# eliotwang/SageAttention

Hardware: AMD Instinct MI355X
Metric: attention fwd TFLOPS at head_dim=128 seqlen=8192 (INT8 QK^T + FP16 PV, quantizers included) (higher is better)
Workload: dtype int8+fp16; 1 GPU; c3: qk_int8_pv_fp16 (B,H,N,D)=(4,32,8192,128) causal=False qk_quant_gran=per_thread; global_batch=4, seq_len=8192, head_dim=128, heads=32, parallelism=single

## Files before the change

### sageattention_amd/csrc/sage_entry.h

```cpp
#pragma once
#include "sage_attn_common.h"

namespace sage {

struct QuantParams {
  const uint16_t* x;
  int64_t xsb, xsh, xsn;
  const uint16_t* mean;
  int8_t* out;
  int64_t osb, osh, osn;
  float* scale;
  const uint16_t* dot_vec;
  float* dot_out;
  int dot_group;
  int N, G;
  int gran, is_key;
  int warp;
  int warp_shift;
  float mult;
  int rounding;
  const int* cu;
  int64_t o_blk, ss_b, ss_h, ss_blk;
  const float* mean_part;
  int S;
  uint16_t* km_out;
};

struct VPrepParams {
  const uint16_t* v;
  int64_t sb, sh, sn;
  uint8_t* out;
  int64_t ob, oh, od, o_tile;
  float* v_scale;
  const float* part;
  float scale_max;
};

struct QuantOptions {
  const int* cu = nullptr;
  int64_t out_blk_stride = 0;
  const int64_t* scale_strides = nullptr;
  const float* mean_part = nullptr;
  int S = 0;
  void* km_out = nullptr;
};

struct QuantCall {
  QuantParams p;
  int B, H, D, blk;
  bool bf16;
};
int quant_check(QuantCall& c, const sage_tensor* x, int dtype, int B, int H, int N, int D, const void* mean,
                const sage_tensor* out, float* scale, int gran, int is_key, int blk, int warp, float mult, int rounding,
                const void* lse_dot_vec, int dot_group, float* lse_dot, const QuantOptions& opt = QuantOptions());
int quant_launch(const QuantCall& c, hipStream_t st);

struct KSmoothCall {
  QuantCall q;
  sage_tensor k;
  float* part;
  int per_wg;
  const int32_t* kv_lens = nullptr;
};
int k_smooth_quant_check(KSmoothCall& c, const sage_tensor* k, int dtype, int B, int H, int N, int D, const sage_tensor* out,
                         float* scale, void* km, int gran, int rounding, void* workspace, const int32_t* kv_lens = nullptr);
int k_smooth_quant_launch(const KSmoothCall& c, hipStream_t st);

struct KVPrepCall {
  QuantCall k;
  VPrepParams v;
  float* kpart;
  float* vpart;
  int nblk_k, nunit_v;
  int per_k, per_v;
  bool streaming;
  const int32_t* kv_lens = nullptr;
};
int kv_prepare_check(KVPrepCall& c, const sage_tensor* k, const sage_tensor* v, int dtype, int B, int H, int N, int D,
                     const sage_tensor* k_int8, float* k_scale, void* km, int gran, int rounding, const sage_tensor* v_fp8,
                     float* v_scale, float scale_max, void* workspace,
                     const int32_t* kv_lens = nullptr);
int kv_prepare_launch(const KVPrepCall& c, hipStream_t st);

struct AttnArgs {
  const sage_tensor *q = nullptr, *k8 = nullptr, *v = nullptr, *o = nullptr;
  bool pv_fp8 = false;
  int v_dtype = SAGE_F16, o_dtype = SAGE_F16;
  const float *q_scale = nullptr, *k_scale = nullptr, *v_scale = nullptr, *v_mean = nullptr;
  float* lse = nullptr;
  int B = 0, Hq = 0, Hk = 0, M = 0, N = 0, D = 0;
  int is_causal = 0, qk_gran = 0, blkq = 0, warpq = 0;
  float sm_scale = 0.f;
  int logit_mult_is_one = 0;
  const int *cu_q = nullptr, *cu_k = nullptr;
  int q_dtype = -1;
  const void* km = nullptr;
  const void* mask = nullptr;
  int mask_kind = 0;
  const int64_t* mask_strides = nullptr;
  const sage_kv_layout* kvl = nullptr;
  int nwaves = 0;
  bool block_sparse = false;
  const int32_t* block_lists = nullptr;
  int64_t block_lists_bytes = 0;
  bool pv_skip = false;
  const float* pv_thresh = nullptr;
  int32_t* pv_skipped = nullptr;
  bool key_lens = false;
  const int32_t* kv_lens = nullptr;
  bool block_key_lens = false;
  const int32_t* block_kv_lens = nullptr;
  bool split_kv = false;
  const int32_t* split_kv_lens = nullptr;
  int num_splits = 0;
  void* split_workspace = nullptr;
  size_t split_workspace_bytes = 0;
};

struct AttnCall {
  AttnParams p;
  int D, nwaves;
  bool pv_fp8, causal, kthread, v_bf16;
  bool sparse;
  bool pvskip;
  bool kvlen;
  bool sparse_kvlen;
  bool splitkv;
};
int attn_check(AttnCall& c, const AttnArgs& a);
int attn_launch(const AttnCall& c, hipStream_t st);
int launch_blocksparse_pvskip(const AttnCall& c, hipStream_t st);
int launch_kvlen(const AttnCall& c, hipStream_t st);
int launch_blocksparse_kvlen(const AttnCall& c, hipStream_t st);
int launch_blocksparse_pvskip_kvlen(const AttnCall& c, hipStream_t st);
int launch_splitkv(const AttnCall& c, hipStream_t st);
inline int64_t splitkv_bytes(int B, int Hq, int M, int D, int S) {
  return (int64_t)S * B * Hq * M * ((int64_t)D + 1) * 4;
}

inline int64_t block_sparse_bytes(int B, int Hq, int M, int N) {
  return (int64_t)B * Hq * (((int64_t)M + 127) / 128) * block_list_row(N) * 4;
}

struct FinishLseCall {
  const float* lse2;
  const float* corr;
  float sm_scale;
  float* out;
  int64_t n;
};
int finish_lse_check(FinishLseCall& c, const float* lse2, const float* corr, float sm_scale, float* lse_out, int64_t n);
int finish_lse_launch(const FinishLseCall& c, hipStream_t st);

}
```

### sageattention_amd/csrc/sage_op.hip

```cpp
#include "sage_entry.h"

namespace {

constexpr size_t kAlign = 256;
inline size_t up(size_t x) { return (x + kAlign - 1) / kAlign * kAlign; }

struct Plan {
  bool fuse_q;
  size_t k8, ks, km, pre_ws, v8, v_scale, q8, qs, corr, lse2, total;
  int gk, gq, npad;
};

bool make_plan(Plan& pl, const sage::AttnArgs& a, bool want_lse, const sage_op_opts* o) {
  const int B = a.B, Hq = a.Hq, Hk = a.Hk, M = a.M, N = a.N, D = a.D;
  if (B <= 0 || Hq <= 0 || Hk <= 0 || M <= 0 || N <= 0 || (D != 64 && D != 128) || !o) return false;
  const int gran = o->qk_gran, warpq = o->warpq ? o->warpq : 32;
  if (gran != SAGE_GRAN_PER_WARP && gran != SAGE_GRAN_PER_THREAD) return false;
  if (warpq != 16 && warpq != 32) return false;
  pl.fuse_q = o->fuse_q != 0;
  pl.npad = (N + 63) / 64 * 64;
  pl.gk = (N + 63) / 64 * (gran == SAGE_GRAN_PER_THREAD ? 4 : 1);
  const int nblkq = (M + 127) / 128;
  pl.gq = gran == SAGE_GRAN_PER_WARP ? nblkq * (128 / warpq) : nblkq * (128 / warpq) * 8;
  size_t off = 0;
  auto take = [&](size_t bytes) { const size_t at = off; off += up(bytes); return at; };
  pl.k8 = take((size_t)B * Hk * N * D);
  pl.ks = take((size_t)B * Hk * pl.gk * 4);
  pl.km = take((size_t)B * Hk * D * 2);
  const size_t pre = a.pv_fp8 ? sage_kv_prepare_fp8_workspace_bytes(B, Hk, N, D) : sage_k_mean_workspace_bytes(B, Hk, N, D);
  pl.pre_ws = take(pre > 4 ? pre : 4);
  pl.v8 = pl.v_scale = 0;
  if (a.pv_fp8) {
    pl.v8 = take((size_t)B * Hk * D * pl.npad);
    pl.v_scale = take((size_t)B * Hk * D * 4);
  }
  pl.q8 = pl.qs = pl.corr = pl.lse2 = 0;
  if (!pl.fuse_q) {
    pl.q8 = take((size_t)B * Hq * M * D);
    pl.qs = take((size_t)B * Hq * pl.gq * 4);
    if (want_lse) {
      pl.corr = take((size_t)B * Hq * M * 4);
      pl.lse2 = take((size_t)B * Hq * M * 4);
    }
  }
  pl.total = off;
  return true;
}

int run(sage::AttnArgs aa, const sage_tensor* k, int dtype, float scale_max, const sage_op_opts* opts, void* workspace,
        size_t workspace_bytes, sage_stream_t stream) {
  const sage_tensor *const q = aa.q, *const v = aa.v;
  float* const lse = aa.lse;
  const int pv_fp8 = aa.pv_fp8, B = aa.B, Hq = aa.Hq, Hk = aa.Hk, M = aa.M, N = aa.N, D = aa.D;
  if (!q || !k || !v || !aa.o || !opts || !workspace) return SAGE_ERR_INVALID_ARGUMENT;
  if (const int s = sage::dim_dtype_status(D, dtype)) return s;
  if (Hk <= 0 || Hq % Hk != 0) return SAGE_ERR_INVALID_ARGUMENT;
  if (!opts->smooth_k) return SAGE_ERR_UNSUPPORTED;
  if (opts->nwaves != 0 && opts->nwaves != 4 && opts->nwaves != 8) return SAGE_ERR_INVALID_ARGUMENT;
  Plan pl;
  if (!make_plan(pl, aa, lse != nullptr, opts)) return SAGE_ERR_INVALID_ARGUMENT;
  if (workspace_bytes < pl.total || !sage::aligned16(workspace)) return SAGE_ERR_INVALID_ARGUMENT;
  char* const ws = static_cast<char*>(workspace);
  const int gran = opts->qk_gran, warpq = opts->warpq ? opts->warpq : 32;
  const int rounding = gran == SAGE_GRAN_PER_THREAD ? SAGE_ROUND_TRITON : SAGE_ROUND_CUDA;
  const int k_gran = gran == SAGE_GRAN_PER_THREAD ? SAGE_GRAN_PER_THREAD : SAGE_GRAN_PER_BLOCK;
  const sage_tensor k8{ws + pl.k8, (int64_t)Hk * N * D, (int64_t)N * D, D};
  float* const ks = reinterpret_cast<float*>(ws + pl.ks);
  void* const km = ws + pl.km;
  sage_tensor v8{nullptr, 0, 0, 0};
  float* v_scale = nullptr;
  sage::KSmoothCall kc;
  sage::KVPrepCall kvc;
  int st;
  if (pv_fp8) {
    v8 = sage_tensor{ws + pl.v8, (int64_t)Hk * D * pl.npad, (int64_t)D * pl.npad, pl.npad};
    v_scale = reinterpret_cast<float*>(ws + pl.v_scale);
    st = sage::kv_prepare_check(kvc, k, v, dtype, B, Hk, N, D, &k8, ks, km, k_gran, rounding, &v8, v_scale, scale_max,
                                ws + pl.pre_ws);
  } else {
    st = sage::k_smooth_quant_check(kc, k, dtype, B, Hk, N, D, &k8, ks, km, k_gran, rounding, ws + pl.pre_ws);
  }
  if (st != SAGE_OK) return st;
  aa.k8 = &k8; aa.k_scale = ks; aa.v_scale = v_scale; aa.v_dtype = pv_fp8 ? SAGE_F16 : dtype; aa.o_dtype = dtype;
  if (pv_fp8) aa.v = &v8;
  aa.qk_gran = gran; aa.blkq = 128; aa.warpq = warpq; aa.nwaves = opts->nwaves;
  sage::AttnCall ac;
  sage::QuantCall qc;
  sage::FinishLseCall fc;
  const sage_tensor q8{ws + pl.q8, (int64_t)Hq * M * D, (int64_t)M * D, D};
  if (pl.fuse_q) {
    aa.q_dtype = dtype; aa.km = km;
    st = sage::attn_check(ac, aa);
  } else {
    float* const qs = reinterpret_cast<float*>(ws + pl.qs);
    float* const corr = lse ? reinterpret_cast<float*>(ws + pl.corr) : nullptr;
    float* const lse2 = lse ? reinterpret_cast<float*>(ws + pl.lse2) : nullptr;
    st = sage::quant_check(qc, q, dtype, B, Hq, M, D, nullptr, &q8, qs, gran, 0, 128, warpq, 1.0f, rounding, lse ? km : nullptr,
                           Hq / Hk, corr);
    aa.q = &q8; aa.q_scale = qs; aa.lse = lse2;
    if (st == SAGE_OK) st = sage::attn_check(ac, aa);
    if (st == SAGE_OK && lse) st = sage::finish_lse_check(fc, lse2, corr, aa.sm_scale, lse, (int64_t)B * Hq * M);
  }
  if (st != SAGE_OK) return st;
  const hipStream_t s = (hipStream_t)stream;
  st = pv_fp8 ? sage::kv_prepare_launch(kvc, s) : sage::k_smooth_quant_launch(kc, s);
  if (st == SAGE_OK && !pl.fuse_q) st = sage::quant_launch(qc, s);
  if (st == SAGE_OK) st = sage::attn_launch(ac, s);
  if (st == SAGE_OK && !pl.fuse_q && lse) st = sage::finish_lse_launch(fc, s);
  return st;
}

}

extern "C" size_t sage_sageattn_workspace_bytes(int pv_fp8, int B, int Hq, int Hk, int M, int N, int D, int want_lse,
                                                const sage_op_opts* opts) {
  sage::AttnArgs a;
  a.pv_fp8 = pv_fp8 != 0; a.B = B; a.Hq = Hq; a.Hk = Hk; a.M = M; a.N = N; a.D = D;
  Plan pl;
  return make_plan(pl, a, want_lse != 0, opts) ? pl.total : 0;
}

extern "C" int sage_sageattn_pv_f16(const sage_tensor* q, const sage_tensor* k, const sage_tensor* v, int dtype,
                                    const sage_tensor* o, float* lse, int B, int Hq, int Hk, int M, int N, int D, int is_causal,
                                    float sm_scale, const sage_op_opts* opts, void* workspace, size_t workspace_bytes,
                                    sage_stream_t stream) {
  sage::AttnArgs a;
  a.q = q; a.v = v; a.o = o; a.lse = lse; a.B = B; a.Hq = Hq; a.Hk = Hk; a.M = M; a.N = N; a.D = D; a.is_causal = is_causal;
  a.sm_scale = sm_scale;
  return run(a, k, dtype, 0.f, opts, workspace, workspace_bytes, stream);
}

extern "C" int sage_sageattn_pv_f8(const sage_tensor* q, const sage_tensor* k, const sage_tensor* v, int dtype,
                                   const sage_tensor* o, float* lse, int B, int Hq, int Hk, int M, int N, int D, int is_causal,
                                   float sm_scale, float scale_max, const sage_op_opts* opts, void* workspace,
                                   size_t workspace_bytes, sage_stream_t stream) {
  if (!(scale_max > 0.f)) return SAGE_ERR_INVALID_ARGUMENT;
  sage::AttnArgs a;
  a.q = q; a.v = v; a.pv_fp8 = true; a.o = o; a.lse = lse; a.B = B; a.Hq = Hq; a.Hk = Hk; a.M = M; a.N = N; a.D = D;
  a.is_causal = is_causal; a.sm_scale = sm_scale;
  return run(a, k, dtype, scale_max, opts, workspace, workspace_bytes, stream);
}
```

### sageattention_amd/csrc/sage_quant.hip

```cpp
#include "sage_entry.h"
#include "sage_fp8_kernels.h"

namespace sage {

constexpr int KMEAN_ROWS = 256;
__host__ __device__ __forceinline__ int kmean_chunk_rows(int N) {
  const int c256 = (N + KMEAN_ROWS - 1) / KMEAN_ROWS;
  return KMEAN_ROWS * ((c256 + 15) / 16 > 0 ? (c256 + 15) / 16 : 1);
}

__host__ __device__ __forceinline__ int kmean_chunks(int N) {
  const int rows = kmean_chunk_rows(N);
  return (N + rows - 1) / rows;
}
__host__ __device__ __forceinline__ int kmean_max_chunks(int N) {
  const int c256 = (N + KMEAN_ROWS - 1) / KMEAN_ROWS;
  return c256 < 16 ? c256 : 16;
}
__device__ __forceinline__ int kv_len_of(const int32_t* __restrict__ kv_lens, int b, int N) { return min(max(kv_lens[b], 0), N); }

template <int D, bool BF16>
__device__ __forceinline__ void k_mean_partial_body(const uint16_t* __restrict__ k, int64_t sb, int64_t sh, int64_t sn, int N,
                                                    float* __restrict__ part, int S, int s, int h, int b, int H,
                                                    float (*red)[D + 1]) {
// ... 373 lines not shown
          y = y + (y >= 0.f ? 0.5f : -0.5f);
          q[j] = min(max((int)y, -128), 127);
        }
        w = make_uint2(pack_i8x4(q[0], q[1], q[2], q[3]), pack_i8x4(q[4], q[5], q[6], q[7]));
      }
    } else {
      uint32_t tb[8];
#pragma unroll
      for (int j = 0; j < 8; ++j) tb[j] = __float_as_uint(xf[i][j] * r + 12582912.f);
      w = make_uint2(pack_i8x4(tb[0], tb[1], tb[2], tb[3]), pack_i8x4(tb[4], tb[5], tb[6], tb[7]));
    }
    if (!RAGGED || row0 + i * RPP < p.N) *reinterpret_cast<uint2*>(obase + (int64_t)(i * RPP) * p.osn) = w;
  }
}

template <int D, bool BF16, bool TRITON, bool PER_THREAD>
__device__ __forceinline__ void k_quant_stream_walk(const QuantParams& p, const int per_wg, const int wg, const int h, const int b,
                                                    const int H, unsigned int (*gmax)[64], float (*mpart)[D]) {
  using G = QuantGeom<D, 64>;
  const int nblk = (p.N + 63) / 64, nfull = p.N / 64;
  const int blk0 = wg * per_wg, blk1 = min(blk0 + per_wg, nblk);
  if (threadIdx.x < 192) (&gmax[0][0])[threadIdx.x] = 0u;
  const uint16_t* xbase = p.x + b * p.xsb + h * p.xsh + (threadIdx.x % G::TPR) * 8;
  uint4 raw[G::NP];
  if (blk0 < nfull) k_load_rows<D, false>(xbase, p.xsn, blk0, p.N, raw);
  else k_load_rows<D, true>(xbase, p.xsn, blk0, p.N, raw);
  const uint4 mbits = quant_mean_bits<D, BF16>(p, h, b, H, wg == 0, mpart);
  int par = 0;
  for (int blk = blk0; blk < blk1; ++blk) {
    unsigned int* const zero_next = gmax[par == 0 ? 2 : par - 1];
    if (blk < nfull) {
      k_quant_block<D, BF16, TRITON, PER_THREAD, false>(p, blk, h, b, raw, mbits, gmax[par], zero_next, [&] {
        if (blk + 1 < blk1) {
          if (blk + 1 < nfull) k_load_rows<D, false>(xbase, p.xsn, blk + 1, p.N, raw);
          else k_load_rows<D, true>(xbase, p.xsn, blk + 1, p.N, raw);
        }
      });
    } else {
      k_quant_block<D, BF16, TRITON, PER_THREAD, true>(p, blk, h, b, raw, mbits, gmax[par], zero_next, [] {});
    }
    par = par == 2 ? 0 : par + 1;
  }
}

template <int D, bool BF16, bool TRITON>
__device__ __forceinline__ void k_quant_stream_body(const QuantParams& p, const int per_wg, const int wg, const int h, const int b,
                                                    const int H, unsigned int (*gmax)[64], float (*mpart)[D]) {
  if (p.gran == SAGE_GRAN_PER_THREAD) k_quant_stream_walk<D, BF16, TRITON, true>(p, per_wg, wg, h, b, H, gmax, mpart);
  else k_quant_stream_walk<D, BF16, TRITON, false>(p, per_wg, wg, h, b, H, gmax, mpart);
}

template <int D, bool BF16, bool TRITON>
__global__ __launch_bounds__(256, D == 64 ? 5 : 4) void k_quant_stream_kernel(const QuantParams p, const int per_wg) {
  __shared__ unsigned int gmax[3][64];
  __shared__ __attribute__((aligned(16))) float mpart[16][D];
  k_quant_stream_body<D, BF16, TRITON>(p, per_wg, blockIdx.x, blockIdx.y, blockIdx.z, gridDim.y, gmax, mpart);
}

template <int D>
__device__ __forceinline__ bool kvlen_batch_params(QuantParams& p, int64_t& part_shift, const int32_t* __restrict__ kv_lens,
                                                   const int blk0, const int h, const int b, const int H, const bool k_half) {
  const int len = kv_len_of(kv_lens, b, p.N);
  if (k_half && len == 0 && blk0 == 0 && threadIdx.x < D / 8)
    *reinterpret_cast<uint4*>(p.km_out + ((int64_t)b * H + h) * D + threadIdx.x * 8) = make_uint4(0u, 0u, 0u, 0u);
  const int slots = kmean_max_chunks(p.N);
  p.N = len;
  p.S = kmean_chunks(len);
  part_shift = ((int64_t)b * H + h) * (slots - p.S) * D;
  p.mean_part += part_shift;
  return blk0 * 64 < len;
}

template <int D, bool BF16, bool TRITON>
__global__ __launch_bounds__(256, D == 64 ? 5 : 4) void k_quant_stream_kvlen_kernel(const QuantParams p, const int per_wg,
                                                                                    const int32_t* __restrict__ kv_lens) {
  __shared__ unsigned int gmax[3][64];
  __shared__ __attribute__((aligned(16))) float mpart[16][D];
  QuantParams pb = p;
  int64_t part_shift;
  if (!kvlen_batch_params<D>(pb, part_shift, kv_lens, blockIdx.x * per_wg, blockIdx.y, blockIdx.z, gridDim.y, true)) return;
  k_quant_stream_body<D, BF16, TRITON>(pb, per_wg, blockIdx.x, blockIdx.y, blockIdx.z, gridDim.y, gmax, mpart);
}


template <int D, bool BF16>
__device__ __forceinline__ void v_amax_partial_body(const uint16_t* __restrict__ v, int64_t sb, int64_t sh, int64_t sn, int N,
                                                    float* __restrict__ part, int S, int s, int h, int b, int H,
                                                    float (*red)[D + 1]) {
  constexpr int TPR = D / 8, RPP = 256 / TPR;
  const int tr = threadIdx.x / TPR, tc = threadIdx.x % TPR;
  const uint16_t* base = v + b * sb + h * sh + tc * 8;
  float am[8] = {0, 0, 0, 0, 0, 0, 0, 0};
  const int rows = kmean_chunk_rows(N);
  if ((s + 1) * rows <= N) {
#pragma unroll 8
    for (int i = 0; i < rows / RPP; ++i) {
      float f[8];
      unpack8<BF16>(*reinterpret_cast<const uint4*>(base + (int64_t)(s * rows + i * RPP + tr) * sn), f);
#pragma unroll
      for (int j = 0; j < 8; ++j) am[j] = fmaxf(am[j], fabsf(f[j]));
    }
  } else {
#pragma unroll 4
    for (int i = 0; i < rows / RPP; ++i) {
      const int row = s * rows + i * RPP + tr;
      if (row < N) {
        float f[8];
        unpack8<BF16>(*reinterpret_cast<const uint4*>(base + (int64_t)row * sn), f);
#pragma unroll
        for (int j = 0; j < 8; ++j) am[j] = fmaxf(am[j], fabsf(f[j]));
      }
    }
  }
#pragma unroll
  for (int j = 0; j < 8; ++j) red[tr][tc * 8 + j] = am[j];
  __syncthreads();
  if (threadIdx.x < D) {
    float a = red[0][threadIdx.x];
    for (int r = 1; r < RPP; ++r) a = fmaxf(a, red[r][threadIdx.x]);
    part[(((int64_t)b * H + h) * S + s) * D + threadIdx.x] = a;
  }
}

template <int D, bool BF16>
__global__ __launch_bounds__(256) void kv_partial_kernel(const uint16_t* __restrict__ k, int64_t ksb, int64_t ksh, int64_t ksn,
                                                         const uint16_t* __restrict__ v, int64_t vsb, int64_t vsh, int64_t vsn,
                                                         int N, float* __restrict__ kpart, float* __restrict__ vpart, int S) {
  static_assert(KMEAN_ROWS == VQ_ROWS, "one chunk size for both tensors");
  __shared__ float red[256 / (D / 8)][D + 1];
  const int x = blockIdx.x;
  if (x < S) k_mean_partial_body<D, BF16>(k, ksb, ksh, ksn, N, kpart, S, x, blockIdx.y, blockIdx.z, gridDim.y, red);
  else v_amax_partial_body<D, BF16>(v, vsb, vsh, vsn, N, vpart, S, x - S, blockIdx.y, blockIdx.z, gridDim.y, red);
}

template <int D, bool BF16>
__global__ __launch_bounds__(256) void kv_partial_kvlen_kernel(const uint16_t* __restrict__ k, int64_t ksb, int64_t ksh, int64_t ksn,
                                                               const uint16_t* __restrict__ v, int64_t vsb, int64_t vsh, int64_t vsn,
                                                               int N, float* __restrict__ kpart, float* __restrict__ vpart, int S,
                                                               const int32_t* __restrict__ kv_lens) {
  __shared__ float red[256 / (D / 8)][D + 1];
  const int len = kv_len_of(kv_lens, blockIdx.z, N);
  const int x = blockIdx.x, s = x < S ? x : x - S;
  if (s >= kmean_chunks(len)) return;
  if (x < S) k_mean_partial_body<D, BF16>(k, ksb, ksh, ksn, len, kpart, S, s, blockIdx.y, blockIdx.z, gridDim.y, red);
  else v_amax_partial_body<D, BF16>(v, vsb, vsh, vsn, len, vpart, S, s, blockIdx.y, blockIdx.z, gridDim.y, red);
}

template <int D, bool BF16>
__device__ __forceinline__ void v_quant_unit(const QuantParams& p, const VPrepParams& q, const int bx, const int h, const int b,
                                             const int H, float (*exch)[D], uint32_t* tile) {
  using G = VQuantGeom<D>;
  const int tg = threadIdx.x / G::TPR, tc = threadIdx.x % G::TPR;
  uint4 raw[4];
  v_quant_load<D>(q.v + b * q.sb + h * q.sh, q.sn, p.N, bx, raw);
  if (tg < p.S) {
    const float* pp = q.part + (((int64_t)b * H + h) * p.S + tg) * D + tc * 8;
    *reinterpret_cast<float4*>(&exch[tg][tc * 8]) = *reinterpret_cast<const float4*>(pp);
    *reinterpret_cast<float4*>(&exch[tg][tc * 8 + 4]) = *reinterpret_cast<const float4*>(pp + 4);
  }
  __syncthreads();
  if (tg == 0) {
    float rc[8], vs[8];
#pragma unroll
    for (int j = 0; j < 8; ++j) {
      float a = exch[0][tc * 8 + j];
      for (int s_ = 1; s_ < p.S; ++s_) a = fmaxf(a, exch[s_][tc * 8 + j]);
      rc[j] = a > 0.f ? q.scale_max / a : 0.f;
      vs[j] = a / q.scale_max;
    }
#pragma unroll
    for (int j = 0; j < 8; ++j) exch[0][tc * 8 + j] = rc[j];
    if (bx == 0) {
      float* o = q.v_scale + ((int64_t)b * H + h) * D + tc * 8;
      *reinterpret_cast<float4*>(o) = make_float4(vs[0], vs[1], vs[2], vs[3]);
      *reinterpret_cast<float4*>(o + 4) = make_float4(vs[4], vs[5], vs[6], vs[7]);
    }
  }
  __syncthreads();
  float mean[8], rcp[8];
#pragma unroll
  for (int j = 0; j < 8; ++j) { mean[j] = 0.f; rcp[j] = exch[0][tc * 8 + j]; }
  v_quant_to_image<D, BF16>(raw, p.N, bx, mean, rcp, tile);
  __syncthreads();
  v_quant_store_image<D>(q.out, q.ob, q.oh, q.od, q.o_tile, p.N, bx, h, b, tile);
}

template <int D, bool BF16, bool TRITON>
__global__ __launch_bounds__(256, D == 64 ? 8 : 7) void kv_quant_kernel(const QuantParams p, const VPrepParams q, const int nblk_k) {
  using G = VQuantGeom<D>;
  __shared__ unsigned int gmax[64];
  __shared__ __attribute__((aligned(16))) float exch[16][D];
  __shared__ __attribute__((aligned(16))) uint32_t tile[G::BLKS * G::IMG];
  const int h = blockIdx.y, b = blockIdx.z, H = gridDim.y;
  if ((int)blockIdx.x < nblk_k) {
    quant_qk_int8_body<D, 64, BF16, TRITON>(p, blockIdx.x, h, b, H, gmax, exch);
    return;
  }
  v_quant_unit<D, BF16>(p, q, blockIdx.x - nblk_k, h, b, H, exch, tile);
}

template <int D, bool BF16, bool TRITON>
__global__ __launch_bounds__(256, D == 64 ? 8 : 7) void kv_quant_kvlen_kernel(const QuantParams p, const VPrepParams q, const int nblk_k,
                                                                              const int32_t* __restrict__ kv_lens) {
  using G = VQuantGeom<D>;
  __shared__ unsigned int gmax[64];
  __shared__ __attribute__((aligned(16))) float exch[16][D];
  __shared__ __attribute__((aligned(16))) uint32_t tile[G::BLKS * G::IMG];
  const int h = blockIdx.y, b = blockIdx.z, H = gridDim.y;
  const bool k_half = (int)blockIdx.x < nblk_k;
  const int unit = k_half ? blockIdx.x : blockIdx.x - nblk_k;
  QuantParams pb = p;
  VPrepParams qb = q;
  int64_t part_shift;
  if (!kvlen_batch_params<D>(pb, part_shift, kv_lens, k_half ? unit : unit * G::BLKS, h, b, H, k_half)) return;
  qb.part += part_shift;
// ... 78 lines not shown
  VPrepParams qb = q;
  int64_t part_shift;
  if (!kvlen_batch_params<D>(pb, part_shift, kv_lens, k_half ? wg * per_k : wg * per_v * G::BLKS, h, b, H, k_half)) return;
  qb.part += part_shift;
  if (k_half) k_quant_stream_body<D, BF16, TRITON>(pb, per_k, wg, h, b, H, gmax, exch);
  else v_quant_stream_walk<D, BF16>(pb, qb, per_v, wg, h, b, H, exch, tile);
}

template <bool BF16>
__global__ __launch_bounds__(256) void sub_mean_f16_kernel(const uint16_t* __restrict__ v, int64_t sb, int64_t sh,
                                                           int64_t sn, const uint16_t* __restrict__ vm,
                                                           uint16_t* __restrict__ out, int64_t ob, int64_t oh,
                                                           int64_t on, int N, int D) {
  const int TPR = D / 8, RPP = 256 / TPR;
  const int h = blockIdx.y, b = blockIdx.z, H = gridDim.y;
  const int tr = threadIdx.x / TPR, tc = threadIdx.x % TPR;
  const int row = blockIdx.x * RPP + tr;
  if (row >= N) return;
  float m[8], x[8];
  unpack8<BF16>(*reinterpret_cast<const uint4*>(vm + ((int64_t)b * H + h) * D + tc * 8), m);
  unpack8<BF16>(*reinterpret_cast<const uint4*>(v + b * sb + h * sh + (int64_t)row * sn + tc * 8), x);
  uint32_t w[4];
#pragma unroll
  for (int j = 0; j < 4; ++j) {
    const float lo = round_to_elem<BF16>(x[2 * j] - m[2 * j]);
    const float hi = round_to_elem<BF16>(x[2 * j + 1] - m[2 * j + 1]);
    w[j] = (uint32_t)f32_to_elem_bits<false>(lo) | ((uint32_t)f32_to_elem_bits<false>(hi) << 16);
  }
  *reinterpret_cast<uint4*>(out + b * ob + h * oh + (int64_t)row * on + tc * 8) = make_uint4(w[0], w[1], w[2], w[3]);
}


static int units_per_wg(int64_t BH, int units, int64_t target, int64_t cap) {
  int64_t per = (BH * units + target - 1) / target;
  per = per > cap ? cap : per;
  return (int)(per < 1 ? 1 : per > units ? units : per);
}

static void launch_k_mean_partial(const sage_tensor& k, int B, int H, int N, int D, bool bf16, float* part, int S,
                                  hipStream_t st) {
  by_dim(D, [&](auto d) {
    by_flag(bf16, [&](auto bf) {
      hipLaunchKernelGGL((k_mean_partial_kernel<decltype(d)::value, decltype(bf)::value>), dim3(S, H, B), dim3(256), 0, st,
                         (const uint16_t*)k.data, k.stride_b, k.stride_h, k.stride_n, N, part, S);
    });
  });
}

int quant_check(QuantCall& c, const sage_tensor* x, int dtype, int B, int H, int N, int D, const void* mean,
                const sage_tensor* out, float* scale, int gran, int is_key, int blk, int warp, float mult, int rounding,
                const void* lse_dot_vec, int dot_group, float* lse_dot, const QuantOptions& opt) {
  if (!tensor_ok(x, 8) || !tensor_ok(out, 8) || !scale || B <= 0 || H <= 0 || N <= 0) return SAGE_ERR_INVALID_ARGUMENT;
  if (const int s = dim_dtype_status(D, dtype)) return s;
  if (gran < SAGE_GRAN_PER_BLOCK || gran > SAGE_GRAN_PER_THREAD) return SAGE_ERR_INVALID_ARGUMENT;
  if (rounding != SAGE_ROUND_TRITON && rounding != SAGE_ROUND_CUDA) return SAGE_ERR_INVALID_ARGUMENT;
  if (blk != 64 && blk != 128) return SAGE_ERR_INVALID_ARGUMENT;
  if (gran == SAGE_GRAN_PER_BLOCK) warp = blk;
  if ((warp != 16 && warp != 32 && warp != 64 && warp != 128) || blk % warp != 0) return SAGE_ERR_INVALID_ARGUMENT;
  if (mean && !aligned16(mean)) return SAGE_ERR_INVALID_ARGUMENT;
  if (opt.mean_part && (opt.S < 1 || opt.S > 16 || !aligned16(opt.mean_part))) return SAGE_ERR_INVALID_ARGUMENT;
  if ((lse_dot_vec != nullptr) != (lse_dot != nullptr)) return SAGE_ERR_INVALID_ARGUMENT;
  if (lse_dot_vec && (dot_group <= 0 || H % dot_group != 0 || !aligned16(lse_dot_vec))) return SAGE_ERR_INVALID_ARGUMENT;
  const int nblk = (N + blk - 1) / blk;
  const int gpb = gran == SAGE_GRAN_PER_BLOCK ? 1 : gran == SAGE_GRAN_PER_WARP ? blk / warp : (blk / warp) * (is_key ? 4 : 8);
  if (gpb > 64) return SAGE_ERR_INVALID_ARGUMENT;
  QuantParams& p = c.p;
  p.x = (const uint16_t*)x->data; p.xsb = x->stride_b; p.xsh = x->stride_h; p.xsn = x->stride_n;
  p.mean = (const uint16_t*)mean;
  p.out = (int8_t*)out->data; p.osb = out->stride_b; p.osh = out->stride_h; p.osn = out->stride_n;
  p.scale = scale; p.dot_vec = (const uint16_t*)lse_dot_vec; p.dot_out = lse_dot; p.dot_group = dot_group > 0 ? dot_group : 1;
  p.cu = opt.cu;
  p.mean_part = opt.mean_part; p.S = opt.S; p.km_out = (uint16_t*)opt.km_out;
  p.o_blk = opt.out_blk_stride ? opt.out_blk_stride : (int64_t)blk * out->stride_n;
  p.ss_b = opt.scale_strides ? opt.scale_strides[0] : (int64_t)H * nblk * gpb;
  p.ss_h = opt.scale_strides ? opt.scale_strides[1] : (int64_t)nblk * gpb;
  p.ss_blk = opt.scale_strides ? opt.scale_strides[2] : gpb;
  if (opt.out_blk_stride < 0 || (opt.out_blk_stride & 7) || p.ss_blk < gpb) return SAGE_ERR_INVALID_ARGUMENT;
  p.N = N; p.G = nblk * gpb; p.gran = gran; p.is_key = is_key ? 1 : 0; p.warp = warp; p.mult = mult; p.rounding = rounding;
  p.warp_shift = warp == 16 ? 4 : warp == 32 ? 5 : warp == 64 ? 6 : 7;
  c.B = B; c.H = H; c.D = D; c.blk = blk; c.bf16 = dtype == SAGE_BF16;
  return SAGE_OK;
}

int quant_launch(const QuantCall& c, hipStream_t st) {
  const dim3 grid((c.p.N + c.blk - 1) / c.blk, c.H, c.B);
  launch_begin();
  by_dim(c.D, [&](auto d) {
    by_flag(c.blk == 128, [&](auto b128) {
      by_flag(c.bf16, [&](auto bf) {
        by_flag(c.p.rounding == SAGE_ROUND_TRITON, [&](auto tr) {
          constexpr int BLK = decltype(b128)::value ? 128 : 64;
          hipLaunchKernelGGL((quant_qk_int8_kernel<decltype(d)::value, BLK, decltype(bf)::value, decltype(tr)::value>), grid,
                             dim3(256), 0, st, c.p);
        });
      });
    });
  });
  return launch_status();
}

int k_smooth_quant_check(KSmoothCall& c, const sage_tensor* k, int dtype, int B, int H, int N, int D, const sage_tensor* out,
                         float* scale, void* km, int gran, int rounding, void* workspace, const int32_t* kv_lens) {
  if (!km || !workspace || (kv_lens && !aligned16(km))) return SAGE_ERR_INVALID_ARGUMENT;
  if (gran != SAGE_GRAN_PER_BLOCK && gran != SAGE_GRAN_PER_THREAD) return SAGE_ERR_INVALID_ARGUMENT;
  if (!tensor_ok(k, 8) || B <= 0 || H <= 0 || N <= 0) return SAGE_ERR_INVALID_ARGUMENT;
  if (const int s = dim_dtype_status(D, dtype)) return s;
  QuantOptions opt;
  opt.mean_part = c.part = (float*)workspace;
  opt.S = kmean_chunks(N);
  opt.km_out = km;
  if (const int s = quant_check(c.q, k, dtype, B, H, N, D, nullptr, out, scale, gran, 1, 64, 64, 1.0f, rounding, nullptr, 1,
                                nullptr, opt))
    return s;
  c.k = *k;
  c.kv_lens = kv_lens;
  const int nblk = (N + 63) / 64;
  c.per_wg = units_per_wg((int64_t)B * H, nblk, 256 * (D == 64 ? 5 : 4), nblk);
  return SAGE_OK;
}

int k_smooth_quant_launch(const KSmoothCall& c, hipStream_t st) {
  const QuantParams& p = c.q.p;
  launch_begin();
  if (c.kv_lens) {
    const int slots = kmean_max_chunks(p.N);
    by_dim(c.q.D, [&](auto d) {
      by_flag(c.q.bf16, [&](auto bf) {
        hipLaunchKernelGGL((k_mean_partial_kvlen_kernel<decltype(d)::value, decltype(bf)::value>), dim3(slots, c.q.H, c.q.B),
                           dim3(256), 0, st, (const uint16_t*)c.k.data, c.k.stride_b, c.k.stride_h, c.k.stride_n, p.N, c.part,
                           slots, c.kv_lens);
      });
    });
  } else {
    launch_k_mean_partial(c.k, c.q.B, c.q.H, p.N, c.q.D, c.q.bf16, c.part, p.S, st);
  }
  if (launch_status() != SAGE_OK) return SAGE_ERR_LAUNCH;
  const int nblk = (p.N + 63) / 64;
  const dim3 grid((nblk + c.per_wg - 1) / c.per_wg, c.q.H, c.q.B);
  launch_begin();
  by_dim(c.q.D, [&](auto d) {
    by_flag(c.q.bf16, [&](auto bf) {
      by_flag(p.rounding == SAGE_ROUND_TRITON, [&](auto tr) {
        constexpr int DD = decltype(d)::value;
        constexpr bool BF = decltype(bf)::value, TR = decltype(tr)::value;
        if (c.kv_lens)
          hipLaunchKernelGGL((k_quant_stream_kvlen_kernel<DD, BF, TR>), grid, dim3(256), 0, st, p, c.per_wg, c.kv_lens);
        else
          hipLaunchKernelGGL((k_quant_stream_kernel<DD, BF, TR>), grid, dim3(256), 0, st, p, c.per_wg);
      });
    });
  });
  return launch_status();
}

int kv_prepare_check(KVPrepCall& c, const sage_tensor* k, const sage_tensor* v, int dtype, int B, int H, int N, int D,
                     const sage_tensor* k_int8, float* k_scale, void* km, int gran, int rounding, const sage_tensor* v_fp8,
                     float* v_scale, float scale_max, void* workspace, const int32_t* kv_lens) {
  if (!km || !workspace || !v_scale || !(scale_max > 0.f)) return SAGE_ERR_INVALID_ARGUMENT;
  if (kv_lens && !aligned16(km)) return SAGE_ERR_INVALID_ARGUMENT;
  if (gran != SAGE_GRAN_PER_BLOCK && gran != SAGE_GRAN_PER_THREAD) return SAGE_ERR_INVALID_ARGUMENT;
  if (!tensor_ok(k, 8) || !tensor_ok(v, 8) || B <= 0 || H <= 0 || N <= 0) return SAGE_ERR_INVALID_ARGUMENT;
  if (!tensor_ok(v_fp8, 16)) return SAGE_ERR_INVALID_ARGUMENT;
  if (const int s = dim_dtype_status(D, dtype)) return s;
  const int S = kmean_chunks(N);
  const int slots = kv_lens ? kmean_max_chunks(N) : S;
  c.kpart = (float*)workspace;
  c.vpart = c.kpart + (size_t)B * H * slots * D;
  c.kv_lens = kv_lens;
  QuantOptions opt;
  opt.mean_part = c.kpart;
  opt.S = S;
  opt.km_out = km;
  if (const int s = quant_check(c.k, k, dtype, B, H, N, D, nullptr, k_int8, k_scale, gran, 1, 64, 64, 1.0f, rounding, nullptr,
                                1, nullptr, opt))
    return s;
  VPrepParams& q = c.v;
  q.v = (const uint16_t*)v->data; q.sb = v->stride_b; q.sh = v->stride_h; q.sn = v->stride_n;
  q.out = (uint8_t*)v_fp8->data; q.ob = v_fp8->stride_b; q.oh = v_fp8->stride_h; q.od = v_fp8->stride_n; q.o_tile = 64;
  q.v_scale = v_scale; q.part = c.vpart; q.scale_max = scale_max;
  c.nblk_k = (N + 63) / 64;
  const int blks = by_dim(D, [](auto d) { return VQuantGeom<decltype(d)::value>::BLKS; });
  c.nunit_v = (c.nblk_k + blks - 1) / blks;
  const int64_t target = 128 * (D == 64 ? 5 : 4), cap = 32;
  c.per_k = units_per_wg((int64_t)B * H, c.nblk_k, target, cap);
  c.per_v = units_per_wg((int64_t)B * H, c.nunit_v, target, cap);
  c.streaming = c.per_v >= (D == 64 ? 4 : 12);
  return SAGE_OK;
}

int kv_prepare_launch(const KVPrepCall& c, hipStream_t st) {
  const QuantParams& p = c.k.p;
  const VPrepParams& q = c.v;
  const int B = c.k.B, H = c.k.H;
  launch_begin();
  by_dim(c.k.D, [&](auto d) {
    by_flag(c.k.bf16, [&](auto bf) {
      constexpr int DD = decltype(d)::value;
      constexpr bool BF = decltype(bf)::value;
      if (c.kv_lens)
        hipLaunchKernelGGL((kv_partial_kvlen_kernel<DD, BF>), dim3(2 * kmean_max_chunks(p.N), H, B), dim3(256), 0, st, p.x, p.xsb,
                           p.xsh, p.xsn, q.v, q.sb, q.sh, q.sn, p.N, c.kpart, c.vpart, kmean_max_chunks(p.N), c.kv_lens);
      else
        hipLaunchKernelGGL((kv_partial_kernel<DD, BF>), dim3(2 * p.S, H, B), dim3(256), 0, st, p.x, p.xsb, p.xsh, p.xsn, q.v,
                           q.sb, q.sh, q.sn, p.N, c.kpart, c.vpart, p.S);
    });
  });
  if (launch_status() != SAGE_OK) return SAGE_ERR_LAUNCH;
  const int nwg_k = (c.nblk_k + c.per_k - 1) / c.per_k, nwg_v = (c.nunit_v + c.per_v - 1) / c.per_v;
  by_dim(c.k.D, [&](auto d) {
    by_flag(c.k.bf16, [&](auto bf) {
      by_flag(p.rounding == SAGE_ROUND_TRITON, [&](auto tr) {
        constexpr int DD = decltype(d)::value;
        constexpr bool BF = decltype(bf)::value, TR = decltype(tr)::value;
        if (c.kv_lens && c.streaming)
          hipLaunchKernelGGL((kv_quant_stream_kvlen_kernel<DD, BF, TR>), dim3(nwg_k + nwg_v, H, B), dim3(256), 0, st, p, q,
                             c.per_k, nwg_k, c.per_v, c.kv_lens);
        else if (c.kv_lens)
          hipLaunchKernelGGL((kv_quant_kvlen_kernel<DD, BF, TR>), dim3(c.nblk_k + c.nunit_v, H, B), dim3(256), 0, st, p, q,
                             c.nblk_k, c.kv_lens);
        else if (c.streaming)
          hipLaunchKernelGGL((kv_quant_stream_kernel<DD, BF, TR>), dim3(nwg_k + nwg_v, H, B), dim3(256), 0, st, p, q, c.per_k,
                             nwg_k, c.per_v);
        else
          hipLaunchKernelGGL((kv_quant_kernel<DD, BF, TR>), dim3(c.nblk_k + c.nunit_v, H, B), dim3(256), 0, st, p, q, c.nblk_k);
      });
    });
  });
  return launch_status();
}

}

using namespace sage;

extern "C" size_t sage_k_mean_workspace_bytes(int B, int H, int N, int D) {
  const size_t S = (size_t)(N + KMEAN_ROWS - 1) / KMEAN_ROWS;
  return (size_t)B * H * S * D * sizeof(float);
}

extern "C" int sage_k_mean(const sage_tensor* k, int dtype, int B, int H, int N, int D, void* km, void* workspace,
                           sage_stream_t stream) {
  if (!tensor_ok(k, 8) || !km || !workspace || B <= 0 || H <= 0 || N <= 0) return SAGE_ERR_INVALID_ARGUMENT;
  if (const int s = dim_dtype_status(D, dtype)) return s;
  const int S = kmean_chunks(N);
  float* const ws = (float*)workspace;
  hipStream_t st = (hipStream_t)stream;
  launch_begin();
  launch_k_mean_partial(*k, B, H, N, D, dtype == SAGE_BF16, ws, S, st);
  by_flag(dtype == SAGE_BF16, [&](auto bf) {
    hipLaunchKernelGGL((k_mean_final_kernel<decltype(bf)::value>), dim3(B * H), dim3(128), 0, st, ws, S, D, N, (uint16_t*)km);
  });
  return launch_status();
}

extern "C" int sage_quant_qk_int8(const sage_tensor* x, int dtype, int B, int H, int N, int D, const void* mean,
                                  const sage_tensor* out, float* scale, int gran, int is_key, int blk, int warp,
                                  float mult, int rounding, const void* lse_dot_vec, int dot_group, float* lse_dot,
                                  sage_stream_t stream) {
  QuantCall c;
  if (const int s = quant_check(c, x, dtype, B, H, N, D, mean, out, scale, gran, is_key, blk, warp, mult, rounding,
                                lse_dot_vec, dot_group, lse_dot))
    return s;
  return quant_launch(c, (hipStream_t)stream);
}

extern "C" int sage_quant_qk_int8_varlen(const sage_tensor* x, int dtype, const int* cu_seqlens, int num_seqs, int H,
                                         int max_seqlen, int D, const void* mean, const sage_tensor* out, float* scale,
                                         int gran, int is_key, int blk, int warp, float mult, int rounding,
                                         sage_stream_t stream) {
  if (!cu_seqlens) return SAGE_ERR_INVALID_ARGUMENT;
  QuantOptions opt;
  opt.cu = cu_seqlens;
  QuantCall c;
  if (const int s = quant_check(c, x, dtype, num_seqs, H, max_seqlen, D, mean, out, scale, gran, is_key, blk, warp, mult,
                                rounding, nullptr, 1, nullptr, opt))
    return s;
  return quant_launch(c, (hipStream_t)stream);
}
// ... 76 lines not shown
```

Before: 1295 TFLOPS.

## Fuse Q quantization into K-mean stats launch and add streaming Q quant kernel

Adds a persistent streaming Q quantization kernel that processes several 64-row units per workgroup, prefetching the next unit's rows while quantizing the current one. When no LSE is needed, Q quantization rides along in the same grid as the K-mean/V-amax partial statistics kernel, removing one kernel launch and letting the two independent phases overlap across CUs. This adds template variants and a more complex grid decomposition, and the fused kernel's shared memory and occupancy are set by the larger of the two bodies.

```diff
diff --git a/sageattention_amd/csrc/sage_entry.h b/sageattention_amd/csrc/sage_entry.h
--- a/sageattention_amd/csrc/sage_entry.h
+++ b/sageattention_amd/csrc/sage_entry.h
@@ -49,11 +49,14 @@
   QuantParams p;
   int B, H, D, blk;
   bool bf16;
+  int per_wg = 0;
 };
 int quant_check(QuantCall& c, const sage_tensor* x, int dtype, int B, int H, int N, int D, const void* mean,
                 const sage_tensor* out, float* scale, int gran, int is_key, int blk, int warp, float mult, int rounding,
                 const void* lse_dot_vec, int dot_group, float* lse_dot, const QuantOptions& opt = QuantOptions());
 int quant_launch(const QuantCall& c, hipStream_t st);
+int q_quant_check(QuantCall& c, const sage_tensor* q, int dtype, int B, int Hq, int Hk, int M, int D, const sage_tensor* out,
+                  float* scale, int gran, int warp, const void* km, float* corr);
 
 struct KSmoothCall {
   QuantCall q;
@@ -64,7 +67,7 @@
 };
 int k_smooth_quant_check(KSmoothCall& c, const sage_tensor* k, int dtype, int B, int H, int N, int D, const sage_tensor* out,
                          float* scale, void* km, int gran, int rounding, void* workspace, const int32_t* kv_lens = nullptr);
-int k_smooth_quant_launch(const KSmoothCall& c, hipStream_t st);
+int k_smooth_quant_launch(const KSmoothCall& c, hipStream_t st, const QuantCall* q_ride = nullptr);
 
 struct KVPrepCall {
   QuantCall k;
@@ -80,7 +83,7 @@
                      const sage_tensor* k_int8, float* k_scale, void* km, int gran, int rounding, const sage_tensor* v_fp8,
                      float* v_scale, float scale_max, void* workspace,
                      const int32_t* kv_lens = nullptr);
-int kv_prepare_launch(const KVPrepCall& c, hipStream_t st);
+int kv_prepare_launch(const KVPrepCall& c, hipStream_t st, const QuantCall* q_ride = nullptr);
 
 struct AttnArgs {
   const sage_tensor *q = nullptr, *k8 = nullptr, *v = nullptr, *o = nullptr;
diff --git a/sageattention_amd/csrc/sage_op.hip b/sageattention_amd/csrc/sage_op.hip
--- a/sageattention_amd/csrc/sage_op.hip
+++ b/sageattention_amd/csrc/sage_op.hip
@@ -45,6 +45,10 @@
   }
   pl.total = off;
   return true;
+}
+
+bool ride_fits(int B, int Hq, int Hk, int M) {
+  return (int64_t)B * Hk * 32 + (int64_t)B * Hq * ((M + 127) / 128 * 2) < ((int64_t)1 << 31);
 }
 
 int run(sage::AttnArgs aa, const sage_tensor* k, int dtype, float scale_max, const sage_op_opts* opts, void* workspace,
@@ -95,16 +99,16 @@
     float* const qs = reinterpret_cast<float*>(ws + pl.qs);
     float* const corr = lse ? reinterpret_cast<float*>(ws + pl.corr) : nullptr;
     float* const lse2 = lse ? reinterpret_cast<float*>(ws + pl.lse2) : nullptr;
-    st = sage::quant_check(qc, q, dtype, B, Hq, M, D, nullptr, &q8, qs, gran, 0, 128, warpq, 1.0f, rounding, lse ? km : nullptr,
-                           Hq / Hk, corr);
+    st = sage::q_quant_check(qc, q, dtype, B, Hq, Hk, M, D, &q8, qs, gran, warpq, km, corr);
     aa.q = &q8; aa.q_scale = qs; aa.lse = lse2;
     if (st == SAGE_OK) st = sage::attn_check(ac, aa);
     if (st == SAGE_OK && lse) st = sage::finish_lse_check(fc, lse2, corr, aa.sm_scale, lse, (int64_t)B * Hq * M);
   }
   if (st != SAGE_OK) return st;
   const hipStream_t s = (hipStream_t)stream;
-  st = pv_fp8 ? sage::kv_prepare_launch(kvc, s) : sage::k_smooth_quant_launch(kc, s);
-  if (st == SAGE_OK && !pl.fuse_q) st = sage::quant_launch(qc, s);
+  const sage::QuantCall* const q_ride = !pl.fuse_q && !lse && qc.per_wg > 0 && ride_fits(B, Hq, Hk, M) ? &qc : nullptr;
+  st = pv_fp8 ? sage::kv_prepare_launch(kvc, s, q_ride) : sage::k_smooth_quant_launch(kc, s, q_ride);
+  if (st == SAGE_OK && !pl.fuse_q && !q_ride) st = sage::quant_launch(qc, s);
   if (st == SAGE_OK) st = sage::attn_launch(ac, s);
   if (st == SAGE_OK && !pl.fuse_q && lse) st = sage::finish_lse_launch(fc, s);
   return st;
diff --git a/sageattention_amd/csrc/sage_quant.hip b/sageattention_amd/csrc/sage_quant.hip
--- a/sageattention_amd/csrc/sage_quant.hip
+++ b/sageattention_amd/csrc/sage_quant.hip
@@ -479,6 +479,140 @@
   k_quant_stream_body<D, BF16, TRITON>(pb, per_wg, blockIdx.x, blockIdx.y, blockIdx.z, gridDim.y, gmax, mpart);
 }
 
+template <int D, int WARP, bool PT>
+struct QStreamGeom {
+  using G = QuantGeom<D, 64>;
+  static_assert(WARP == 16 || WARP == 32, "16- or 32-row scale groups");
+  static_assert(!PT || WARP == 32, "per_thread: 32-row warp groups");
+  static constexpr int PPG = WARP > G::RPP ? WARP / G::RPP : 1;
+  static constexpr int NS = G::NP / PPG;
+  static constexpr int GPU = (64 / WARP) * (PT ? 8 : 1);
+  static_assert(G::RPP % 8 == 0 && (G::RPP % WARP == 0 || WARP % G::RPP == 0), "a pass lies in one group per thread");
+};
+
+template <int D, bool BF16, int WARP, bool PT, bool LSE, bool RAGGED, typename AfterPhase1>
+__device__ __forceinline__ void q_quant_unit(const QuantParams& p, const int u, const int h, const int b, const int H,
+                                             uint4 (&raw)[QuantGeom<D, 64>::NP], unsigned int* gmax, unsigned int* zero_next,
+                                             AfterPhase1 after_phase1) {
+  using G = QuantGeom<D, 64>;
+  using Q = QStreamGeom<D, WARP, PT>;
+  constexpr int TPR = G::TPR, RPP = G::RPP, NP = G::NP, PPG = Q::PPG, NS = Q::NS;
+  const int tr = (int)threadIdx.x / TPR, tc = (int)threadIdx.x % TPR;
+  const int row0 = u * 64 + tr;
+  float xf[NP][8];
+  float dvec[8];
+  if constexpr (LSE) {
+    const int Hk = H / p.dot_group;
+    unpack8<BF16>(*reinterpret_cast<const uint4*>(p.dot_vec + ((int64_t)b * Hk + h / p.dot_group) * D + tc * 8), dvec);
+  }
+#pragma unroll
+  for (int s = 0; s < NS; ++s) {
+    float amax = 0.f;
+#pragma unroll
+    for (int t = 0; t < PPG; ++t) {
+      const int i = s * PPG + t;
+      unpack8<BF16>(raw[i], xf[i]);
+      const bool valid = !RAGGED || row0 + i * RPP < p.N;
+      if constexpr (LSE) {
+        float dot = 0.f;
+#pragma unroll
+        for (int j = 0; j < 8; ++j) dot += xf[i][j] * dvec[j];
+#pragma unroll
+        for (int o = 1; o < TPR; o <<= 1) dot += __shfl_xor(dot, o);
+        if (tc == 0 && valid) p.dot_out[((int64_t)b * H + h) * p.N + row0 + i * RPP] = dot;
+      }
+      float am = RAGGED ? 0.f : amax;
+#pragma unroll
+      for (int j = 0; j < 8; ++j) am = fmaxf(am, fabsf(xf[i][j]));
+      if constexpr (RAGGED) amax = fmaxf(amax, valid ? am : 0.f);
+      else amax = am;
+    }
+    amax = row_lanes_max<TPR>(amax);
+    const int lr0 = s * PPG * RPP + tr;
+    if (tc == 0) atomicMax(&gmax[PT ? (lr0 / WARP) * 8 + (tr & 7) : lr0 / WARP], __float_as_uint(amax));
+  }
+  after_phase1();
+  __syncthreads();
+  if (threadIdx.x < Q::GPU) zero_next[threadIdx.x] = 0u;
+
+  int8_t* obase = p.out + b * p.osb + h * p.osh + (u >> 1) * p.o_blk + (int64_t)((u & 1) * 64 + tr) * p.osn + tc * 8;
+  float* sbase = p.scale + b * p.ss_b + h * p.ss_h + (u >> 1) * p.ss_blk + (u & 1) * Q::GPU;
+#pragma unroll
+  for (int s = 0; s < NS; ++s) {
+    const int lr0 = s * PPG * RPP + tr;
+    const int g = PT ? (lr0 / WARP) * 8 + (tr & 7) : lr0 / WARP;
+    const bool first = tc == 0 && (PT ? (lr0 & (WARP - 1)) < 8 : (lr0 & (WARP - 1)) == 0);
+    const float a = __uint_as_float(gmax[g]);
+    const float sc = PT ? a / 127.f + 0.0000001f : 0.f;
+    const float r = PT ? 1.0f / sc : 127.f / fmaxf(a, 0.0000001f);
+    if (first) sbase[g] = PT ? sc : fmaxf(a, 0.0000001f) / 127.f;
+    const bool r_unusable = PT && !(fabsf(r) < 3.0e38f);
+#pragma unroll
+    for (int t = 0; t < PPG; ++t) {
+      const int i = s * PPG + t;
+      uint2 w;
+      if constexpr (PT) {
+        bool near;
+        w = round_half_away_pack8(xf[i], r, near);
+        if (__builtin_amdgcn_ballot_w64(near || r_unusable) != 0) {
+          int q[8];
+#pragma unroll
+          for (int j = 0; j < 8; ++j) {
+            float y = xf[i][j] / sc;
+            y = y + (y >= 0.f ? 0.5f : -0.5f);
+            q[j] = min(max((int)y, -128), 127);
+          }
+          w = make_uint2(pack_i8x4(q[0], q[1], q[2], q[3]), pack_i8x4(q[4], q[5], q[6], q[7]));
+        }
+      } else {
+        uint32_t tb[8];
+#pragma unroll
+        for (int j = 0; j < 8; ++j) tb[j] = __float_as_uint(xf[i][j] * r + 12582912.f);
+        w = make_uint2(pack_i8x4(tb[0], tb[1], tb[2], tb[3]), pack_i8x4(tb[4], tb[5], tb[6], tb[7]));
+      }
+      if (!RAGGED || row0 + i * RPP < p.N) *reinterpret_cast<uint2*>(obase + (int64_t)(i * RPP) * p.osn) = w;
+    }
+  }
+}
+
+__host__ __device__ __forceinline__ int q_units(int N) { return (N + 127) / 128 * 2; }
+
+template <int D, bool BF16, int WARP, bool PT, bool LSE>
+__device__ __forceinline__ void q_quant_stream_body(const QuantParams& p, const int per_wg, const int wg, const int h, const int b,
+                                                    const int H, unsigned int (*gmax)[64]) {
+  using G = QuantGeom<D, 64>;
+  const int nfull = p.N / 64;
+  const int u0 = wg * per_wg, u1 = min(u0 + per_wg, q_units(p.N));
+  if (threadIdx.x < 192) (&gmax[0][0])[threadIdx.x] = 0u;
+  const uint16_t* xbase = p.x + b * p.xsb + h * p.xsh + (threadIdx.x % G::TPR) * 8;
+  uint4 raw[G::NP];
+  if (u0 < nfull) k_load_rows<D, false>(xbase, p.xsn, u0, p.N, raw);
+  else k_load_rows<D, true>(xbase, p.xsn, u0, p.N, raw);
+  __syncthreads();
+  int par = 0;
+  for (int u = u0; u < u1; ++u) {
+    unsigned int* const zero_next = gmax[par == 0 ? 2 : par - 1];
+    if (u < nfull) {
+      q_quant_unit<D, BF16, WARP, PT, LSE, false>(p, u, h, b, H, raw, gmax[par], zero_next, [&] {
+        if (u + 1 < u1) {
+          if (u + 1 < nfull) k_load_rows<D, false>(xbase, p.xsn, u + 1, p.N, raw);
+          else k_load_rows<D, true>(xbase, p.xsn, u + 1, p.N, raw);
+        }
+      });
+    } else {
+      q_quant_unit<D, BF16, WARP, PT, LSE, true>(p, u, h, b, H, raw, gmax[par], zero_next, [] {});
+      if (u + 1 < u1) k_load_rows<D, true>(xbase, p.xsn, u + 1, p.N, raw);
+    }
+    par = par == 2 ? 0 : par + 1;
+  }
+}
+
+template <int D, bool BF16, int WARP, bool PT, bool LSE>
+__global__ __launch_bounds__(256, D == 64 ? 5 : 4) void q_quant_stream_kernel(const QuantParams p, const int per_wg) {
+  __shared__ unsigned int gmax[3][64];
+  q_quant_stream_body<D, BF16, WARP, PT, LSE>(p, per_wg, blockIdx.x, blockIdx.y, blockIdx.z, gridDim.y, gmax);
+}
+
 
 template <int D, bool BF16>
 __device__ __forceinline__ void v_amax_partial_body(const uint16_t* __restrict__ v, int64_t sb, int64_t sh, int64_t sn, int N,
@@ -528,6 +662,26 @@
   const int x = blockIdx.x;
   if (x < S) k_mean_partial_body<D, BF16>(k, ksb, ksh, ksn, N, kpart, S, x, blockIdx.y, blockIdx.z, gridDim.y, red);
   else v_amax_partial_body<D, BF16>(v, vsb, vsh, vsn, N, vpart, S, x - S, blockIdx.y, blockIdx.z, gridDim.y, red);
+}
+
+template <int D, bool BF16, int WARP, bool PT, bool WITH_V>
+__global__ __launch_bounds__(256, D == 64 ? 5 : 4) void stats_q_quant_kernel(
+    const uint16_t* __restrict__ k, int64_t ksb, int64_t ksh, int64_t ksn, const uint16_t* __restrict__ v, int64_t vsb, int64_t vsh,
+    int64_t vsn, int N, float* __restrict__ kpart, float* __restrict__ vpart, int S, int Hk, int n_stat, const QuantParams p,
+    const int per_wg, const int nwg_q, const int Hq) {
+  __shared__ float red[256 / (D / 8)][D + 1];
+  __shared__ unsigned int gmax[3][64];
+  int x = blockIdx.x;
+  if (x < n_stat) {
+    const int SS = WITH_V ? 2 * S : S;
+    const int s = x % SS, bh = x / SS, h = bh % Hk, b = bh / Hk;
+    if (!WITH_V || s < S) k_mean_partial_body<D, BF16>(k, ksb, ksh, ksn, N, kpart, S, s, h, b, Hk, red);
+    else v_amax_partial_body<D, BF16>(v, vsb, vsh, vsn, N, vpart, S, s - S, h, b, Hk, red);
+    return;
+  }
+  x -= n_stat;
+  const int wg = x % nwg_q, bh = x / nwg_q;
+  q_quant_stream_body<D, BF16, WARP, PT, false>(p, per_wg, wg, bh % Hq, bh / Hq, Hq, gmax);
 }
 
 template <int D, bool BF16>
@@ -772,9 +926,45 @@
   return SAGE_OK;
 }
 
+int q_quant_check(QuantCall& c, const sage_tensor* q, int dtype, int B, int Hq, int Hk, int M, int D, const sage_tensor* out,
+                  float* scale, int gran, int warp, const void* km, float* corr) {
+  if (gran != SAGE_GRAN_PER_WARP && gran != SAGE_GRAN_PER_THREAD) return SAGE_ERR_INVALID_ARGUMENT;
+  if ((warp != 16 && warp != 32) || Hk <= 0 || Hq % Hk != 0) return SAGE_ERR_INVALID_ARGUMENT;
+  const int rounding = gran == SAGE_GRAN_PER_THREAD ? SAGE_ROUND_TRITON : SAGE_ROUND_CUDA;
+  if (const int s = quant_check(c, q, dtype, B, Hq, M, D, nullptr, out, scale, gran, 0, 128, warp, 1.0f, rounding,
+                                corr ? km : nullptr, Hq / Hk, corr))
+    return s;
+  c.per_wg = 0;
+  if (gran == SAGE_GRAN_PER_THREAD && warp != 32) return SAGE_OK;
+  c.per_wg = units_per_wg((int64_t)B * Hq, q_units(M), 256 * (D == 64 ? 5 : 4), q_units(M));
+  return SAGE_OK;
+}
+
+template <class F>
+static void by_q_form(const QuantCall& c, F&& f) {
+  by_flag(c.p.dot_vec != nullptr, [&](auto lse) {
+    if (c.p.gran == SAGE_GRAN_PER_THREAD) f(std::integral_constant<int, 32>{}, std::true_type{}, lse);
+    else if (c.p.warp == 16) f(std::integral_constant<int, 16>{}, std::false_type{}, lse);
+    else f(std::integral_constant<int, 32>{}, std::false_type{}, lse);
+  });
+}
+
 int quant_launch(const QuantCall& c, hipStream_t st) {
+  launch_begin();
+  if (c.per_wg > 0) {
+    const dim3 grid((q_units(c.p.N) + c.per_wg - 1) / c.per_wg, c.H, c.B);
+    by_dim(c.D, [&](auto d) {
+      by_flag(c.bf16, [&](auto bf) {
+        by_q_form(c, [&](auto w, auto pt, auto lse) {
+          hipLaunchKernelGGL((q_quant_stream_kernel<decltype(d)::value, decltype(bf)::value, decltype(w)::value,
+                                                    decltype(pt)::value, decltype(lse)::value>),
+                             grid, dim3(256), 0, st, c.p, c.per_wg);
+        });
+      });
+    });
+    return launch_status();
+  }
   const dim3 grid((c.p.N + c.blk - 1) / c.blk, c.H, c.B);
-  launch_begin();
   by_dim(c.D, [&](auto d) {
     by_flag(c.blk == 128, [&](auto b128) {
       by_flag(c.bf16, [&](auto bf) {
@@ -787,6 +977,25 @@
     });
   });
   return launch_status();
+}
+
+static void launch_stats_q_quant(const QuantParams& pk, int B, int Hk, int D, bool bf16, float* kpart, const VPrepParams* v,
+                                 float* vpart, const QuantCall& qc, hipStream_t st) {
+  const int nwg_q = (q_units(qc.p.N) + qc.per_wg - 1) / qc.per_wg;
+  const int n_stat = (v ? 2 : 1) * pk.S * Hk * B;
+  const dim3 grid((unsigned)(n_stat + nwg_q * qc.H * qc.B));
+  by_dim(D, [&](auto d) {
+    by_flag(bf16, [&](auto bf) {
+      by_flag(v != nullptr, [&](auto wv) {
+        by_q_form(qc, [&](auto w, auto pt, auto) {
+          hipLaunchKernelGGL((stats_q_quant_kernel<decltype(d)::value, decltype(bf)::value, decltype(w)::value, decltype(pt)::value,
+                                                   decltype(wv)::value>),
+                             grid, dim3(256), 0, st, pk.x, pk.xsb, pk.xsh, pk.xsn, v ? v->v : nullptr, v ? v->sb : 0, v ? v->sh : 0,
+                             v ? v->sn : 0, pk.N, kpart, vpart, pk.S, Hk, n_stat, qc.p, qc.per_wg, nwg_q, qc.H);
+        });
+      });
+    });
+  });
 }
 
 int k_smooth_quant_check(KSmoothCall& c, const sage_tensor* k, int dtype, int B, int H, int N, int D, const sage_tensor* out,
@@ -809,10 +1018,12 @@
   return SAGE_OK;
 }
 
-int k_smooth_quant_launch(const KSmoothCall& c, hipStream_t st) {
+int k_smooth_quant_launch(const KSmoothCall& c, hipStream_t st, const QuantCall* q_ride) {
   const QuantParams& p = c.q.p;
   launch_begin();
-  if (c.kv_lens) {
+  if (q_ride) {
+    launch_stats_q_quant(p, c.q.B, c.q.H, c.q.D, c.q.bf16, c.part, nullptr, nullptr, *q_ride, st);
+  } else if (c.kv_lens) {
     const int slots = kmean_max_chunks(p.N);
     by_dim(c.q.D, [&](auto d) {
       by_flag(c.q.bf16, [&](auto bf) {
@@ -878,12 +1089,13 @@
   return SAGE_OK;
 }
 
-int kv_prepare_launch(const KVPrepCall& c, hipStream_t st) {
+int kv_prepare_launch(const KVPrepCall& c, hipStream_t st, const QuantCall* q_ride) {
   const QuantParams& p = c.k.p;
   const VPrepParams& q = c.v;
   const int B = c.k.B, H = c.k.H;
   launch_begin();
-  by_dim(c.k.D, [&](auto d) {
+  if (q_ride) launch_stats_q_quant(p, B, H, c.k.D, c.k.bf16, c.kpart, &q, c.vpart, *q_ride, st);
+  else by_dim(c.k.D, [&](auto d) {
     by_flag(c.k.bf16, [&](auto bf) {
       constexpr int DD = decltype(d)::value;
       constexpr bool BF = decltype(bf)::value;
```

New measurement: 1291 TFLOPS. No clear change (-0.3%).
